# markokr/libacm

Measured on AMD Instinct MI355X. Metric: decoded PCM Msamples/sec over a batch of ACM streams (hot path on HBM-resident staged input), higher is better.
Workload: dtype int32

## Files before the change

### libacm_amd/csrc/acm_kernels.hip

```cpp
#include <hip/hip_runtime.h>

#include <utility>

#include "acm_device.h"

#ifndef ACM_L14_GROUPS
#define ACM_L14_GROUPS 3, 3, 3, 3, 2
#endif
#ifndef ACM_L13_GROUPS
#define ACM_L13_GROUPS 2, 3, 3, 3, 2
#endif

#ifndef ACM_OUT_F32
#define ACM_OUT_F32 0
#endif
#if ACM_OUT_F32
#define ACM_K_EMIT acm_sw_emit_f32
#define ACM_K_SMALL acm_small_level_f32
#define ACM_K_FUSED acm_fused_tile_f32
#define ACM_K_TILE2 acm_f32_tile2
#define ACM_K_CHUNK acm_f32_chunk
#define ACMK_OUT(name) name##_f32
#else
#define ACM_K_EMIT acm_sw_emit
#define ACM_K_SMALL acm_small_level
#define ACM_K_FUSED acm_fused_tile
#define ACM_K_TILE2 acm_tile2
#define ACM_K_CHUNK acm_chunk
#define ACMK_OUT(name) name
#endif

namespace {

__device__ __forceinline__ uint32_t pcm16(int32_t v, int level, unsigned fmt)
{
	uint32_t w = (uint32_t)(v >> level);
	if (fmt & 2u)
		w += 0x8000u;
	w &= 0xFFFFu;
	if (fmt & 1u)
		w = ((w & 0xFFu) << 8) | (w >> 8);
	return w;
}

typedef float v2f __attribute__((ext_vector_type(2)));
typedef float v4f __attribute__((ext_vector_type(4)));

__device__ __forceinline__ v2f pcm_pair_f32(uint32_t w)
{
	const v2f f = { (float)(int32_t)(int16_t)(w & 0xFFFFu), (float)((int32_t)w >> 16) };
	return f * 0x1p-15f;
}

__device__ __forceinline__ v4f pcm_quad_f32(uint32_t a, uint32_t b)
{
	const v2f x = pcm_pair_f32(a), y = pcm_pair_f32(b);
	return v4f{ x.x, x.y, y.x, y.y };
}

__device__ __forceinline__ float pcm_one_f32(int32_t v, int level)
{
	return (float)(int32_t)(int16_t)(uint16_t)pcm16(v, level, ACMHIP_FMT_S16LE) * 0x1p-15f;
}

constexpr int SW_THREADS = 256;

#if !ACM_OUT_F32
__global__ void __launch_bounds__(SW_THREADS)
acm_sw_unpack(const AcmDevStream *__restrict__ streams, const uint32_t *__restrict__ list,
	      const int16_t *__restrict__ idx, const acmhip_blkhdr *__restrict__ hdr,
	      int32_t *__restrict__ x, const uint32_t shift)
{
	const AcmDevStream s = streams[list[blockIdx.y]];
	const uint64_t first = (uint64_t)s.halo_row << s.level;
	const uint64_t n = ((uint64_t)(s.nrows - s.halo_row)) << s.level;
	const int16_t *src = idx + s.idx_off + first;
	const acmhip_blkhdr *h = hdr + s.hdr_off;
	int32_t *dst = x + s.scratch_off;
	for (uint64_t e = (uint64_t)blockIdx.x * SW_THREADS + threadIdx.x; e < n;
	     e += (uint64_t)gridDim.x * SW_THREADS) {
		const uint32_t row = s.halo_row + (uint32_t)(e >> s.level);
		const uint32_t val = h[row / s.rows].val;
		dst[e] = (int32_t)((uint32_t)(int32_t)src[e] * (val << shift));
	}
}

__global__ void __launch_bounds__(SW_THREADS)
// ... 1878 lines not shown
			return (i & 3u) + CB * ((i >> 2) & 1u) + 4u * (i >> 3);
	}

	struct Raw { v4u_t lo[NG][NX], hi[NG][NX]; };
	struct Desc { uint32_t e[NE]; };
	struct Tables {
		v4i_t coef[3][NM][64];
		int32_t bias[3][2][QN];
		int32_t rsum[3][QN];
	};

	static __device__ __forceinline__ void fill_tables(Tables &t, const int tid, const int nthreads)
	{
		constexpr int32_t ONE = 1 << OutScale<L>::SHIFT;
		for (int k = tid; k < 3 * NM * 64; k += nthreads) {
			const int j = k / (NM * 64), mt = (k / 64) % NM, lane = k % 64;
			t.coef[j][mt][lane] = *reinterpret_cast<const v4i_t *>(&ACM_TZ6[VARIANT][j][16 * mt + (lane & 15)][16 * (lane >> 4)]);
		}
		for (int k = tid; k < 3 * 2 * QN; k += nthreads) {
			const int var = k / (2 * QN), par = (k / QN) & 1, q = k % QN;
			t.bias[var][par][q] = par ? 0 : ACM_TZ6_BIAS[VARIANT][var][q] * ONE;
		}
		for (int k = tid; k < 3 * QN; k += nthreads) {
			int32_t sum = 0;
			for (int c = 0; c < 64; c++)
				sum += ACM_TZ6[VARIANT][k / QN][k % QN][c];
			t.rsum[k / QN][k % QN] = 128 * sum;
		}
	}

	static __device__ __forceinline__ Desc fetch_desc(const uint32_t *__restrict__ pairs, const AcmTile2 &r)
	{
		Desc d;
		const uint32_t at = __builtin_amdgcn_readfirstlane((uint32_t)r.idx_off);
#pragma unroll
		for (int j = 0; j < NE; j++)
			d.e[j] = pairs[at + j];
		return d;
	}

	static __device__ __forceinline__ uint32_t entry_of(const Desc &d, const uint32_t u)
	{
		uint32_t e = (uint32_t)opaque_s((int32_t)d.e[0]);
#pragma unroll
		for (int j = 1; j < NE; j++)
			e = (u >> 1) >= (uint32_t)j ? (uint32_t)opaque_s((int32_t)d.e[j]) : e;
		return e;
	}

	static constexpr bool HISTORY_IN_REGISTERS = RR == 1;
#ifndef ACM_K3_DPP_HISTORY
#define ACM_K3_DPP_HISTORY 1
#endif
	static constexpr bool HISTORY_BY_DPP = ACM_K3_DPP_HISTORY && RR >= 2 && NSW == 2 && RR * SIGMA == 16 && SIGMA >= 4;
	static constexpr bool KEEPS_ROWS = HISTORY_IN_REGISTERS || HISTORY_BY_DPP;
	template <int CTRL, int BANKS>
	static __device__ __forceinline__ v4u_t dpp4(const v4u_t old, const v4u_t src)
	{
		v4u_t r;
#pragma unroll
		for (int v = 0; v < 4; v++)
			r[v] = (uint32_t)__builtin_amdgcn_update_dpp((int)old[v], (int)src[v], CTRL, 0xF, BANKS, false);
		return r;
	}
	static constexpr int DPP_W0_BANKS = (1 << (SIGMA / 4)) - 1;
	static __device__ __forceinline__ void hand_history_on(Raw &raw)
	{
#pragma unroll
		for (int k = 0; k < 2; k++) {
			raw.lo[0][k] = dpp4<0x100 + (16 - SIGMA), DPP_W0_BANKS>(raw.lo[0][k], raw.lo[0][k + NSW]);
			raw.hi[0][k] = dpp4<0x100 + (16 - SIGMA), DPP_W0_BANKS>(raw.hi[0][k], raw.hi[0][k + NSW]);
		}
	}
	static __device__ __forceinline__ void take_history_from_partner(Raw &raw)
	{
#pragma unroll
		for (int k = 0; k < 2; k++) {
			raw.lo[0][k] = dpp4<0x110 + SIGMA, 0xF & ~DPP_W0_BANKS>(raw.lo[0][k], raw.lo[0][k + NSW]);
			raw.hi[0][k] = dpp4<0x110 + SIGMA, 0xF & ~DPP_W0_BANKS>(raw.hi[0][k], raw.hi[0][k + NSW]);
		}
	}
	static constexpr int JM = (TR & 1) ? 1 : TR / 2;
	static_assert(JM + 1 <= NE, "entries in reach are entries fetched");
	static __device__ __forceinline__ uint32_t half_bytes(const uint32_t cls) { return (0x4234u >> (4u * cls)) & 15u; }
	template <int J0>
	static __device__ __forceinline__ uint32_t mode_of(const uint32_t flags, const Desc &d, const uint32_t sval)
	{
		const uint32_t cls = d.e[0] & 3u;
		const uint32_t pair_units = (uint32_t)(COLS / 64) * half_bytes(cls);
		bool ok = (flags & ACM_TILE_ONEBLOCK) != 0 && cls != 0u;
		if constexpr (OutScale<L>::SHIFT != 0)
			ok = ok && sval < 65536u;
#pragma unroll
		for (int j = 1; j <= JM; j++)
			ok = ok && (d.e[j] & 3u) == cls;
#pragma unroll
		for (int j = J0; j < JM; j++)
			ok = ok && (d.e[j + 1] >> 2) - (d.e[j] >> 2) == pair_units;
		return ok ? (cls == ACMHIP_BP_NIB12 ? 3u : cls - (ACMHIP_BP_BYTE - 1u)) : 0u;
	}

#ifndef ACM_K3_LD_MOD
#define ACM_K3_LD_MOD " nt"
#endif
	template <bool KEEP>
	static __device__ __forceinline__ void issue(Raw &raw, const uint8_t *arena, const Desc &d, const int lane, const uint32_t odd, const uint32_t mode)
	{
		static_assert(!KEEP || KEEPS_ROWS, "the rows in front belong to another lane");
		constexpr int K0 = KEEP ? 2 : 0, J0 = KEEP ? 1 : 0;
		const uint32_t i = (uint32_t)lane & 15u, ks = (uint32_t)lane >> 4;
		const uint32_t c = class_of(i), rr = RR == 1 ? 0u : i / SIGMA;
		const uint32_t smode = __builtin_amdgcn_readfirstlane(mode);
		uint32_t va[NX][NG], vh[NX][NG];
		const uint8_t *sb[NX][NG];
		if (mode) {
			const uint32_t hb = smode == 1u ? 2u : smode == 2u ? 4u : 3u;
			const uint64_t base = reinterpret_cast<uint64_t>(arena) + ((uint64_t)(d.e[J0] >> 2) << 6);
			const uint32_t vl = (rr * (uint32_t)(NSW * COLS / 2) + c * (uint32_t)(QN / 2)) * hb + 16u * ks;
			const uint32_t vlh = vl - (smode == 3u ? 8u * ks : 0u);
#pragma unroll
			for (int k = K0; k < NX; k++)
#pragma unroll
				for (int g = 0; g < NG; g++) {
					va[k][g] = vl;
					vh[k][g] = vlh;
					sb[k][g] = sgpr_u64(base + (uint64_t)((((TR & 1 ? odd : 0u) + (uint32_t)(k - K0)) * (uint32_t)(COLS / 2) + group_at(g) * (uint32_t)(QN / 2)) * hb));
				}
		} else {
			const uint32_t e0 = d.e[0];
			const uint8_t *base = sgpr_u64(reinterpret_cast<uint64_t>(arena) + ((uint64_t)(e0 >> 2) << 6));
#pragma unroll
			for (int k = K0; k < NX; k++) {
				const uint32_t u = (TR & 1 ? odd : 0u) + rr * NSW + k;
				const uint32_t e = entry_of(d, u);
				const uint32_t hb = half_bytes(e & 3u);
				const uint32_t row_at = (((e >> 2) - (e0 >> 2)) << 6) + ((u & 1u) ? (uint32_t)(COLS / 2) * hb : 0u) + 16u * ks;
#pragma unroll
				for (int g = 0; g < NG; g++) {
					va[k][g] = row_at + (group_at(g) + c) * (uint32_t)(QN / 2) * hb;
					vh[k][g] = va[k][g] - ((e & 3u) == ACMHIP_BP_NIB12 ? 8u * ks : 0u);
					sb[k][g] = base;
				}
			}
		}
#pragma unroll
		for (int k = K0; k < NX; k++)
#pragma unroll
			for (int g = 0; g < NG; g++) {
				if constexpr (KEEPS_ROWS) {
					asm volatile("global_load_dwordx4 %0, %1, %2" ACM_K3_LD_MOD : "=v"(raw.lo[g][k]) : "v"(va[k][g]), "s"(sb[k][g]) : "memory");
					asm volatile("s_cmp_eq_u32 %3, 1\n\ts_cbranch_scc1 .Lacm_z8_%=\n\t"
						     "global_load_dwordx4 %0, %1, %2 offset:64" ACM_K3_LD_MOD "\n"
						     ".Lacm_z8_%=:"
						     : "+v"(raw.hi[g][k]) : "v"(vh[k][g]), "s"(sb[k][g]), "s"(smode) : "memory", "scc");
				} else {
					asm volatile("global_load_dwordx4 %0, %1, %2" : "=v"(raw.lo[g][k]) : "v"(va[k][g]), "s"(sb[k][g]) : "memory");
					asm volatile("s_cmp_eq_u32 %3, 1\n\ts_cbranch_scc1 .Lacm_z8_%=\n\t"
						     "global_load_dwordx4 %0, %1, %2 offset:64\n"
						     ".Lacm_z8_%=:"
						     : "+v"(raw.hi[g][k]) : "v"(vh[k][g]), "s"(sb[k][g]), "s"(smode) : "memory", "scc");
				}
			}
	}
	static __device__ __forceinline__ v4u_t expand_nib(const v4u_t x)
	{
		const uint32_t M = 0xF0F0F0F0u;
		return v4u_t{ x[0] & M, (x[0] << 4) & M, x[1] & M, (x[1] << 4) & M };
	}
	static __device__ __forceinline__ v4u_t sra4(const v4u_t x)
	{
		v4u_t r;
#pragma unroll
		for (int v = 0; v < 4; v++) {
			const uint32_t m = x[v] & 0x80808080u;
			r[v] = ((x[v] >> 4) & 0x0F0F0F0Fu) | ((m << 1) - (m >> 3));
		}
		return r;
	}
	static __device__ __forceinline__ v4u_t shl4(const v4u_t x)
	{
		return v4u_t{ (x[0] << 4) & 0xF0F0F0F0u, (x[1] << 4) & 0xF0F0F0F0u, (x[2] << 4) & 0xF0F0F0F0u, (x[3] << 4) & 0xF0F0F0F0u };
	}
	static __device__ __forceinline__ void shift_history(Raw &raw)
	{
#pragma unroll
		for (int g = 0; g < NG; g++)
#pragma unroll
			for (int k = 0; k < 2; k++) {
				raw.lo[g][k] = raw.lo[g][k + NSW];
				raw.hi[g][k] = raw.hi[g][k + NSW];
			}
	}
	static __device__ __forceinline__ void zero_history(Raw &raw)
	{
		const v4u_t z = { 0, 0, 0, 0 };
#pragma unroll
		for (int g = 0; g < NG; g++)
#pragma unroll
			for (int k = 0; k < 2; k++)
				raw.lo[g][k] = raw.hi[g][k] = z;
	}

	static __device__ __forceinline__ v4i_t mfma(const v4u_t data, const v4i_t coef, const v4i_t acc)
	{
		return __builtin_amdgcn_mfma_i32_16x16x64_i8((v4i_t)data, coef, acc, 0, 0, 0);
	}

	static __device__ __forceinline__ int32_t opaque_s(int32_t v)
	{
		asm("" : "+s"(v));
		return v;
	}
	static __device__ __forceinline__ int32_t opaque_v(int32_t v)
	{
		asm("" : "+v"(v));
		return v;
	}

	template <bool WORDS, bool FAST, bool NIB = false>
	static __device__ __forceinline__ void run_t(const Raw &raw, uint32_t *const tile, const Tables &t, const int lane, const uint32_t hvs,
						     const uint32_t in_front, const uint32_t sval, const bool wordu = false, const Desc *dd = nullptr,
						     const uint32_t odd = 0u, const bool nform = false)
	{
		static_assert(!NIB || (WORDS && FAST), "rows in N form are a fast-path matter; the general path takes them to bytes first");
		const v4i_t zero = { 0, 0, 0, 0 };
		const uint32_t h = (uint32_t)lane >> 4, qd = (uint32_t)lane & 15u;
		uint32_t c0[NH], rrd[NH];
		uint32_t o_lane[NH];
#pragma unroll
		for (int hf = 0; hf < NH; hf++) {
			const uint32_t i = 4u * h + (uint32_t)(hf * NVH);
			c0[hf] = RR == 1 ? class_of(i) : i % SIGMA;
			rrd[hf] = RR == 1 ? 0u : i / SIGMA;
			const uint32_t m_lane = rrd[hf] * (uint32_t)(NSW * COLS) + c0[hf] + (uint32_t)SIGMA * qd;
			o_lane[hf] = m_lane + (m_lane >> PS);
		}
		uint32_t bias_at[NSW][NH];
		int32_t val[NSW][NH], dv2[NSW][NH], dv1[NSW][NH];
		bool step2[NSW], step1[NSW];
		bool small[NSW];
#pragma unroll
		for (int s = 0; s < NSW; s++)
			small[s] = OutScale<L>::SHIFT == 0;
		if constexpr (FAST) {
#pragma unroll
			for (int s = 0; s < NSW; s++) {
				step2[s] = step1[s] = false;
				small[s] = true;
#pragma unroll
				for (int hf = 0; hf < NH; hf++)
					val[s][hf] = dv2[s][hf] = dv1[s][hf] = 0;
			}
		} else if constexpr (RR <= 2) {
			int32_t rowval[TR + 2];
#pragma unroll
			for (int k = 0; k < TR + 2; k++)
				rowval[k] = (int32_t)__builtin_amdgcn_readlane(hvs, k);
#pragma unroll
			for (int s = 0; s < NSW; s++) {
				const int32_t a0 = rowval[s + 2], a1 = rowval[s + 1], a2 = rowval[s];
				if constexpr (RR == 1) {
					val[s][0] = a0;
					dv2[s][0] = a1 - a0;
					dv1[s][0] = a2 - a1;
					step2[s] = a1 != a0;
					step1[s] = a2 != a1;
					small[s] = (uint32_t)a0 < 65536u;
				} else {
					const int32_t b0 = rowval[NSW + s + 2], b1 = rowval[NSW + s + 1], b2 = rowval[NSW + s];
					val[s][0] = rrd[0] ? b0 : a0;
					dv2[s][0] = rrd[0] ? b1 - b0 : a1 - a0;
					dv1[s][0] = rrd[0] ? b2 - b1 : a2 - a1;
					step2[s] = a1 != a0 || b1 != b0;
					step1[s] = a2 != a1 || b2 != b1;
					small[s] = (uint32_t)(a0 | b0) < 65536u;
				}
			}
		} else {
			const uint32_t first = (uint32_t)__builtin_amdgcn_readfirstlane(hvs);
			const bool one_val = __builtin_amdgcn_ballot_w64(lane < TR + 2 && hvs != first) == 0;
#pragma unroll
			for (int s = 0; s < NSW; s++)
				step2[s] = step1[s] = false;
#pragma unroll
			for (int hf = 0; hf < NH; hf++) {
				int32_t g[NSW + 2];
#pragma unroll
				for (int k = 0; k < NSW + 2; k++)
					g[k] = one_val ? (int32_t)first : __builtin_amdgcn_ds_bpermute((int)(4u * (rrd[hf] * NSW + (uint32_t)k)), (int32_t)hvs);
#pragma unroll
				for (int s = 0; s < NSW; s++) {
					val[s][hf] = g[s + 2];
					dv2[s][hf] = g[s + 1] - g[s + 2];
					dv1[s][hf] = g[s] - g[s + 1];
					if (!one_val) {
						step2[s] = step2[s] || __builtin_amdgcn_ballot_w64(dv2[s][hf] != 0) != 0;
						step1[s] = step1[s] || __builtin_amdgcn_ballot_w64(dv1[s][hf] != 0) != 0;
					}
				}
			}
		}
#pragma unroll
		for (int s = 0; s < NSW; s++)
#pragma unroll
			for (int hf = 0; hf < NH; hf++) {
				const uint32_t row = in_front + rrd[hf] * NSW + s;
				bias_at[s][hf] = ((row < 2 ? row : 2u) * 2u + (c0[hf] == 0 ? 0u : 1u)) * (uint32_t)QN + qd;
			}
		const v4i_t *cf = &t.coef[0][0][lane];
		const auto &hi = raw.hi;
#ifndef ACM_K3_MT_UNROLL
#define ACM_K3_MT_UNROLL 1
#endif
#define ACM_PRAGMA_(x) _Pragma(#x)
#define ACM_UNROLL(n) ACM_PRAGMA_(unroll n)
		ACM_UNROLL(ACM_K3_MT_UNROLL)
		for (int mt = 0; mt < NM; mt++) {
			const v4i_t cf0 = cf[0], cf1 = cf[NM * 64], cf2 = cf[2 * NM * 64];
#pragma unroll
			for (int e = 0; e < NSET; e++) {
				const int g = e / NSW, s = e % NSW;
				int32_t b[NH];
#pragma unroll
				for (int hf = 0; hf < NH; hf++)
					b[hf] = g == 0 ? (&t.bias[0][0][0])[bias_at[s][hf] + 16u * (uint32_t)mt] : 0;
				const v4i_t l1 = mfma(raw.lo[g][s], cf2, zero);
				const v4i_t l2 = mfma(raw.lo[g][s + 1], cf1, l1);
				const v4i_t la = mfma(raw.lo[g][s + 2], cf0, l2);
				v4i_t y;
				if constexpr (FAST) {
					const int32_t sv = opaque_s((int32_t)__builtin_amdgcn_readfirstlane(sval));
#pragma unroll
					for (int v = 0; v < 4; v++)
						y[v] = __mul24(la[v], sv) + (v % NVH == 0 ? b[v / NVH] : 0);
					if constexpr (WORDS) {
						const v4i_t h1 = mfma(hi[g][s], cf2, zero);
						const v4i_t h2 = mfma(hi[g][s + 1], cf1, h1);
						const v4i_t ha = mfma(hi[g][s + 2], cf0, h2);
						if constexpr (NIB) {
							const int32_t sv4 = opaque_s((int32_t)__builtin_amdgcn_readfirstlane(sval << 4));
#pragma unroll
							for (int v = 0; v < 4; v++)
								y[v] = __mul24(ha[v], sv4) + y[v];
						} else {
							const uint32_t sv8 = (uint32_t)opaque_s((int32_t)__builtin_amdgcn_readfirstlane(sval << 8));
#pragma unroll
							for (int v = 0; v < 4; v++)
								y[v] = (int32_t)(__umul24((uint32_t)ha[v], sv8) + (uint32_t)y[v]);
						}
					}
				} else {
#pragma unroll
				for (int v = 0; v < 4; v++)
					y[v] = __mul24(la[v], val[s][v / NVH]) + (v % NVH == 0 ? b[v / NVH] : 0);
				if (step2[s]) {
#pragma unroll
					for (int v = 0; v < 4; v++)
						y[v] += __mul24(l2[v], dv2[s][v / NVH]);
				}
				if (step1[s]) {
#pragma unroll
					for (int v = 0; v < 4; v++)
						y[v] += __mul24(l1[v], dv1[s][v / NVH]);
				}
				if constexpr (WORDS && NH == 1) {
					if (wordu) {
						const int32_t *rs = &t.rsum[0][0] + 16 * mt + (int)qd;
						bool urow[3];
#pragma unroll
						for (int j = 0; j < 3; j++)
							urow[j] = (entry_of(*dd, (TR & 1 ? odd : 0u) + rrd[0] * NSW + (uint32_t)(s + j)) & 3u) == ACMHIP_BP_WORDU;
						const int32_t v0 = val[s][0], v1 = v0 + dv2[s][0], v2 = v1 + dv1[s][0];
						const int32_t add = __mul24(urow[2] ? v0 : 0, rs[0]) + __mul24(urow[1] ? v1 : 0, rs[QN]) + __mul24(urow[0] ? v2 : 0, rs[2 * QN]);
#pragma unroll
						for (int v = 0; v < 4; v++)
							y[v] += add;
					}
				}
				if constexpr (WORDS) {
					const v4i_t h1 = mfma(hi[g][s], cf2, zero);
					const v4i_t h2 = mfma(hi[g][s + 1], cf1, h1);
					const v4i_t ha = mfma(hi[g][s + 2], cf0, h2);
					{
						if (small[s] && !step2[s] && !step1[s] && !nform) {
							uint32_t v8[NH];
#pragma unroll
							for (int hf = 0; hf < NH; hf++)
								v8[hf] = (uint32_t)opaque_v((int32_t)((uint32_t)val[s][hf] << 8));
#pragma unroll
							for (int v = 0; v < 4; v++)
								y[v] = (int32_t)(__umul24((uint32_t)ha[v], v8[v / NVH]) + (uint32_t)y[v]);
							goto joined;
						}
					}
					{
					v4i_t yh;
					int32_t wv[NH], w2[NH], w1[NH];
#pragma unroll
					for (int hf = 0; hf < NH; hf++) {
						wv[hf] = opaque_v(val[s][hf]);
						w2[hf] = opaque_v(dv2[s][hf]);
						w1[hf] = opaque_v(dv1[s][hf]);
					}
#pragma unroll
					for (int v = 0; v < 4; v++)
						yh[v] = __mul24(ha[v], wv[v / NVH]);
					if (step2[s]) {
#pragma unroll
						for (int v = 0; v < 4; v++)
							yh[v] += __mul24(h2[v], w2[v / NVH]);
					}
					if (step1[s]) {
#pragma unroll
						for (int v = 0; v < 4; v++)
							yh[v] += __mul24(h1[v], w1[v / NVH]);
					}
					const uint32_t hs = nform ? 4u : 8u;
#pragma unroll
					for (int v = 0; v < 4; v++)
						y[v] = (int32_t)(((uint32_t)opaque_v(yh[v]) << hs) + (uint32_t)y[v]);
					}
				joined:;
				}
				}
				static_assert(COLS % (1 << PS) == 0 && (SIGMA * 16) % (1 << PS) == 0 &&
					      (NG == 1 || (group_at(NG - 1) % (1 << PS) + CB + 7 < (1 << PS) && SIGMA % (1 << PS) == 0)), "address split");
#pragma unroll
				for (int hf = 0; hf < NH; hf++) {
					uint32_t *const o = tile + (o_lane[hf] + (uint32_t)((s * COLS + ((s * COLS) >> PS)) + (group_at(g) + (group_at(g) >> PS))));
#pragma unroll
					for (int v = 0; v < NVH; v++)
						o[v] = (uint32_t)y[hf * NVH + v];
				}
			}
			cf += 64;
#pragma unroll
			for (int hf = 0; hf < NH; hf++)
				o_lane[hf] += SIGMA * 16 + ((SIGMA * 16) >> PS);
		}
	}

	static __device__ __forceinline__ void run(Raw &raw, uint32_t *const tile, const Tables &t, const int lane_, const uint32_t hvs,
						   const Desc &d, const uint32_t in_front, const uint32_t odd, const uint32_t mode, const uint32_t sval,
						   const bool first)
	{
#ifdef ACM_K3_OPAQUE_LANE
		const int lane = opaque_v(lane_);
#else
		const int lane = lane_;
#endif
		const bool all_new = !KEEPS_ROWS || first;
		if (mode == 3u) {
#pragma unroll
			for (int k = 0; k < NX; k++)
				if (k >= 2 || all_new) {
#pragma unroll
					for (int g = 0; g < NG; g++)
						raw.hi[g][k] = expand_nib(raw.hi[g][k]);
				}
			if constexpr (HISTORY_BY_DPP)
				take_history_from_partner(raw);
			run_t<true, true, true>(raw, tile, t, lane, 0u, in_front, sval);
			return;
		}
		if (mode) {
			if constexpr (HISTORY_BY_DPP)
				take_history_from_partner(raw);
			if (mode == 2u)
				run_t<true, true>(raw, tile, t, lane, 0u, in_front, sval);
			else
				run_t<false, true>(raw, tile, t, lane, 0u, in_front, sval);
			return;
		}
		uint32_t any_word = 0, any_nib = 0, any_wordu = 0;
#pragma unroll
		for (int j = 0; j < NE; j++) {
			any_word |= (d.e[j] & 3u) == ACMHIP_BP_WORD ? 1u : 0u;
			any_nib |= (d.e[j] & 3u) == ACMHIP_BP_NIB12 ? 1u : 0u;
			any_wordu |= (d.e[j] & 3u) == ACMHIP_BP_WORDU ? 1u : 0u;
		}
		any_word |= any_wordu;
		const uint32_t rr = RR == 1 ? 0u : ((uint32_t)lane & 15u) / SIGMA;
		if (any_nib) {
#pragma unroll
			for (int k = 0; k < NX; k++)
				if (k >= 2 || all_new) {
					if ((entry_of(d, (TR & 1 ? odd : 0u) + rr * NSW + k) & 3u) == ACMHIP_BP_NIB12) {
#pragma unroll
						for (int g = 0; g < NG; g++)
							raw.hi[g][k] = expand_nib(raw.hi[g][k]);
					}
				}
		}
		if constexpr (HISTORY_BY_DPP)
			take_history_from_partner(raw);
		const bool nform = any_nib && !any_word;
		if (any_word | any_nib) {
#pragma unroll
			for (int k = 0; k < NX; k++) {
				const uint32_t cls = entry_of(d, (TR & 1 ? odd : 0u) + rr * NSW + k) & 3u;
				const uint32_t mask = cls == ACMHIP_BP_BYTE ? 0u : 0xFFFFFFFFu;
#pragma unroll
				for (int g = 0; g < NG; g++)
					raw.hi[g][k] &= mask;
				if (any_nib && !nform && cls == ACMHIP_BP_NIB12) {
#pragma unroll
					for (int g = 0; g < NG; g++)
						raw.hi[g][k] = sra4(raw.hi[g][k]);
				}
			}
			run_t<true, false>(raw, tile, t, lane, hvs, in_front, 0u, any_wordu != 0, &d, odd, nform);
			if (any_nib && !nform && KEEPS_ROWS) {
#pragma unroll
				for (int k = NSW; k < NX; k++)
					if ((entry_of(d, (TR & 1 ? odd : 0u) + rr * NSW + k) & 3u) == ACMHIP_BP_NIB12) {
#pragma unroll
						for (int g = 0; g < NG; g++)
							raw.hi[g][k] = shl4(raw.hi[g][k]);
					}
			}
		} else {
			run_t<false, false>(raw, tile, t, lane, hvs, in_front, 0u);
		}
	}
};

template <int L_, int ABL, int... Gs>
__global__ void __launch_bounds__(64 * FirstPassZ<L_>::NW, 1)
ACM_K_CHUNK(const AcmTile2 *__restrict__ tiles, const uint32_t ntiles, const int16_t *__restrict__ idx, const uint32_t *__restrict__ pairs,
	  const acmhip_blkhdr *__restrict__ hdr, int16_t *__restrict__ pcm, int16_t *__restrict__ sink, const unsigned fmt)
{
	constexpr bool F32 = ACM_OUT_F32;

	using FP = FirstPassZ<L_>;
	using C = typename FP::C;
	constexpr int L = L_, COLS = C::COLS, NELEM = C::NELEM, TR = C::TR, NJ_LAST = C::NJ_LAST, NW = FP::NW;
	constexpr int WTILE = 8 + NELEM + (NELEM >> C::PS);
	constexpr int NCARRY_WORDS = carry_total<C, FP::G, Gs...>();
	constexpr int PASS_ABL = ABL | MODE_WAVE | (FP::NG > 1 && NW == 16 ? MODE_LEAN : 0);

	__shared__ uint32_t tile_mem[NW][WTILE];
	__shared__ uint32_t carry_all[NW][NCARRY_WORDS];
	__shared__ typename FP::Tables tables;

	const int lane0 = threadIdx.x & 63;
	const uint32_t wave = __builtin_amdgcn_readfirstlane(threadIdx.x >> 6);
	FP::fill_tables(tables, threadIdx.x, NW * 64);
	__syncthreads();

	uint32_t *const tile = tile_mem[wave] + 8;
	uint32_t *const carry_mem = carry_all[wave];

	const uint32_t nvw = gridDim.x * NW, vw = blockIdx.x * NW + wave;
	const uint32_t per = (ntiles + nvw - 1) / nvw;
	uint32_t t = vw * per;
	const uint32_t t_end = t + per < ntiles ? t + per : ntiles;
	if (t >= t_end)
		return;
	bool discard = false;
	{
		const uint32_t f0 = tiles[__builtin_amdgcn_readfirstlane(t)].flags;
		if (f0 & ACM_TILE_DISCARD) {
			discard = true;
		} else if (!(f0 & ACM_TILE_FRESH)) {
			discard = true;
			t--;
		}
	}

	auto rows_in_front = [](const AcmTile2 &r) -> uint32_t { return (r.flags & ACM_TILE_FRESH) ? 0u : (r.flags & ACM_TILE_ROW1) ? 1u : 2u; };
	auto fetch_val = [&](const AcmTile2 &r, const int lane, uint32_t v, const uint32_t mode) -> uint32_t {
		const uint32_t *p = &hdr[0].val;
		if (!mode) {
			const uint32_t lr_fetch = (uint32_t)(lane < TR + 2 ? lane : TR + 1);
			const uint32_t missing = 2u - rows_in_front(r);
			const uint32_t q = r.rowpos + (lr_fetch < missing ? 0u : lr_fetch - missing);
			const uint32_t b = r.magic ? __umulhi(q, r.magic) : q;
			p = &hdr[r.hdr_blk + b].val;
		}
		asm volatile("s_cmp_lg_u32 %2, 0\n\ts_cbranch_scc1 .Lacm_zv_%=\n\t"
			     "global_load_dword %0, %1, off\n"
			     ".Lacm_zv_%=:"
			     : "+v"(v) : "v"(p), "s"(__builtin_amdgcn_readfirstlane(mode)) : "memory", "scc");
		return v;
	};
	typedef const uint32_t __attribute__((address_space(4))) *const_u32_ptr;
	auto val_of = [&](const AcmTile2 &r) -> uint32_t {
		const uint64_t a = reinterpret_cast<uint64_t>(&hdr[__builtin_amdgcn_readfirstlane(r.hdr_blk)].val);
		return *(const_u32_ptr)a << OutScale<L>::SHIFT;
	};

	constexpr int NVEC = TR * COLS / 8, PER_OWNER = NJ_LAST / 8, NSTORE = NVEC / 64;
	static_assert(NVEC % 64 == 0, "whole rounds");
	const uint8_t *const arena = reinterpret_cast<const uint8_t *>(idx);
	auto record_at = [&](const uint32_t k) -> AcmTile2 { return tiles[__builtin_amdgcn_readfirstlane(k < t_end ? k : t_end - 1)]; };
	constexpr int MODE_J0 = FP::KEEPS_ROWS ? 1 : 0;
#ifdef ACM_K3_NO_FAST
	auto mode_of = [&](const AcmTile2 &, const typename FP::Desc &, const uint32_t) -> uint32_t { return 0u; };
#else
	auto mode_of = [&](const AcmTile2 &r, const typename FP::Desc &d, const uint32_t sval) -> uint32_t {
		return FP::template mode_of<MODE_J0>(r.flags, d, sval);
	};
#endif
	AcmTile2 cur = record_at(t);
	typename FP::Desc dcur = FP::fetch_desc(pairs, cur);
	typename FP::Raw raw;
	{
		const v4u_t z = { 0, 0, 0, 0 };
#pragma unroll
		for (int g = 0; g < FP::NG; g++)
#pragma unroll
			for (int k = 0; k < FP::NX; k++)
				raw.hi[g][k] = z;
	}
	uint32_t mode_cur = 0u, sv_cur = val_of(cur);
	uint32_t hv = fetch_val(cur, lane0, 0u, 0u);
	FP::template issue<false>(raw, arena, dcur, lane0, (cur.flags & ACM_TILE_ODD) ? 1u : 0u, 0u);
	k2_wait<0>();
	bool fresh = true, first_of_run = true;
	AcmTile2 nxt = record_at(t + 1), nx2 = record_at(t + 2);
	typename FP::Desc dnxt = FP::fetch_desc(pairs, nxt);
	uint32_t sv_nxt = val_of(nxt);
	uint32_t mode_nxt = mode_of(nxt, dnxt, sv_nxt);
#ifdef ACM_STAMPS
	unsigned long long acc_[8] = { 0, 0, 0, 0, 0, 0, 0, 0 };
	unsigned long long last_ = stamp_now();
#endif
	for (;;) {
		const uint32_t tn = t + 1;
		const bool more = tn < t_end;
		int lane = lane0;
#ifdef ACM_K3_OPAQUE_LANE
		asm volatile("" : "+v"(lane));
#endif
		if (fresh)
			for (int k = lane; k < NCARRY_WORDS; k += 64)
				carry_mem[k] = 0u;
		const uint32_t hvs = hv << OutScale<L>::SHIFT;
		ACM_STAMP(0);
		phase_prio<true, PRIO_FIRST_PASS>();
		FP::run(raw, tile, tables, lane, hvs, dcur, rows_in_front(cur), (cur.flags & ACM_TILE_ODD) ? 1u : 0u, mode_cur, sv_cur, first_of_run);
		first_of_run = false;
		phase_prio<true, PRIO_IDLE>();
		ACM_STAMP(1);

		hv = fetch_val(nxt, lane, hv, mode_nxt);
		if constexpr (FP::HISTORY_IN_REGISTERS) {
			FP::shift_history(raw);
			if (nxt.flags & ACM_TILE_FRESH)
				FP::zero_history(raw);
			FP::template issue<true>(raw, arena, dnxt, lane, (nxt.flags & ACM_TILE_ODD) ? 1u : 0u, mode_nxt);
		} else if constexpr (FP::HISTORY_BY_DPP) {
			FP::hand_history_on(raw);
			if (nxt.flags & ACM_TILE_FRESH)
				FP::zero_history(raw);
			FP::template issue<true>(raw, arena, dnxt, lane, (nxt.flags & ACM_TILE_ODD) ? 1u : 0u, mode_nxt);
		} else {
			FP::template issue<false>(raw, arena, dnxt, lane, (nxt.flags & ACM_TILE_ODD) ? 1u : 0u, mode_nxt);
		}
		const AcmTile2 nx3 = record_at(t + 3);
		const typename FP::Desc dnx2 = FP::fetch_desc(pairs, nx2);
		const uint32_t sv_nx2 = val_of(nx2);
		ACM_STAMP(2);
		phase_prio<true, PRIO_LDS_PASSES>();
		run_lds_passes<C, PASS_ABL, true, FP::G, Gs...>(tile, lane, F32 ? (unsigned)ACMHIP_FMT_S16LE : fmt, carry_mem);
		tile_barrier<MODE_WAVE>();
		ACM_STAMP(3);
		if constexpr (F32) {
			float *out = discard ? reinterpret_cast<float *>(sink) : reinterpret_cast<float *>(pcm) + cur.pcm_off;
			lean_store_f32<C, 64, NSTORE, ABL>(tile, lane, out);
		} else {
			typedef uint32_t v4u __attribute__((ext_vector_type(4)));
			v4u *out = discard ? reinterpret_cast<v4u *>(sink) : reinterpret_cast<v4u *>(reinterpret_cast<uint16_t *>(pcm) + cur.pcm_off);
#pragma unroll
			for (int k = 0; k < NSTORE; k++) {
				const int vec = lane + k * 64;
				const uint32_t *q = tile + lds_at<C::PS>((vec / PER_OWNER) * NJ_LAST) + (vec % PER_OWNER) * park_piece<NJ_LAST>();
				const v4u o = { q[0], q[1], q[2], q[3] };
#ifdef ACM_K3_ST_MOD
				asm volatile("global_store_dwordx4 %0, %1, %2" ACM_K3_ST_MOD :: "v"((uint32_t)(vec * 16)), "v"(o), "s"(sgpr_u64(reinterpret_cast<uint64_t>(out))) : "memory");
#else
				__builtin_nontemporal_store(o, &out[vec]);
#endif
			}
		}
		ACM_STAMP(5);
		phase_prio<true, PRIO_IDLE>();
		k2_wait<F32 ? 2 * NSTORE : NSTORE>();
		ACM_STAMP(6);
		tile_barrier<MODE_WAVE>();
		if (!more)
			break;
		fresh = (nxt.flags & (ACM_TILE_FRESH | ACM_TILE_DISCARD)) != 0;
		discard = (nxt.flags & ACM_TILE_DISCARD) != 0;
		cur = nxt;
		dcur = dnxt;
		sv_cur = sv_nxt;
		mode_cur = mode_nxt;
		t = tn;
		nxt = nx2;
		dnxt = dnx2;
		sv_nxt = sv_nx2;
		mode_nxt = mode_of(nxt, dnxt, sv_nxt);
		nx2 = nx3;
	}
#ifdef ACM_STAMPS
	if (lane0 == 0 && vw < 2048)
		for (int k = 0; k < 8; k++)
			g_acm_stamps[vw][k] = acc_[k];
#endif
}

struct Tile2Entry {
	typedef void (*Fn)(const AcmTile2 *, uint32_t, const int16_t *, const uint32_t *, const acmhip_blkhdr *, int16_t *, int16_t *, unsigned);
	Fn fn;
	int threads, tile_rows, wg_per_cu;
};
template <class C, int... Gs>
constexpr Tile2Entry entry_k2()
{
	return Tile2Entry{ ACM_K_TILE2<C, 4, 0, false, Gs...>, C::NT, C::TR, 1024 / C::NT };
}
template <class C, int WPC, int... Gs>
constexpr Tile2Entry entry_k2w()
{
	return Tile2Entry{ ACM_K_TILE2<C, WPC * C::NT / 256, 0, false, Gs...>, C::NT, C::TR, WPC };
}
#ifdef ACM_ABLATION
template <int ABL>
constexpr Tile2Entry abl_k2() { return Tile2Entry{ ACM_K_TILE2<TileCfg<9, 256, 8192>, 4, ABL, false, 3, 3, 3>, 256, 16, 4 }; }
const struct { int mask; Tile2Entry e; } g_tile2_abl[] = {
	{ 1, abl_k2<1>() }, { 2, abl_k2<2>() }, { 4, abl_k2<4>() }, { 6, abl_k2<6>() }, { 8, abl_k2<8>() }, { 16, abl_k2<16>() },
	{ 17, abl_k2<17>() }, { 23, abl_k2<23>() }, { 32, abl_k2<32>() }, { 25, abl_k2<25>() }, { 31, abl_k2<31>() }, { 12, abl_k2<12>() },
};
#endif
const Tile2Entry g_tile2[ACM_K2_MAX_LEVEL - ACM_K2_MIN_LEVEL + 1] = {
	entry_k2<TileCfg<6, 256, 8192>, 2, 2, 2>(),
	entry_k2<TileCfg<7, 256, 8192>, 3, 2, 2>(),
	entry_k2<TileCfg<8, 256, 8192>, 3, 3, 2>(),
	entry_k2<TileCfg<9, 256, 8192>, 3, 3, 3>(),
	entry_k2<TileCfg<10, 256, 8192>, 3, 3, 2, 2>(),
	entry_k2<TileCfg<11, 256, 8192>, 3, 3, 3, 2>(),
	entry_k2w<TileCfg<12, 512, 16384>, 2, 3, 3, 3, 3>(),
	entry_k2w<TileCfg<13, 1024, 32768>, 1, ACM_L13_GROUPS>(),
	entry_k2w<TileCfg<14, 1024, 32768>, 1, ACM_L14_GROUPS>(),
};
inline const Tile2Entry &tile2_entry(uint32_t level)
{
	return g_tile2[level - ACM_K2_MIN_LEVEL];
}
template <class C, int... Gs>
constexpr Tile2Entry entry_k2m()
{
	return Tile2Entry{ ACM_K_TILE2<C, 4, 0, true, Gs...>, C::NT, C::TR, 1024 / C::NT };
}
template <class C, int WPC, int... Gs>
constexpr Tile2Entry entry_k2mw()
{
	return Tile2Entry{ ACM_K_TILE2<C, WPC * C::NT / 256, 0, true, Gs...>, C::NT, C::TR, WPC };
}
#ifndef ACM_K2M_L11
#define ACM_K2M_L11 entry_k2m<TileCfg<11, 256, 8192>, 4, 3, 2, 2>(), 4
#endif
#ifndef ACM_K2M_L12
#define ACM_K2M_L12 entry_k2mw<TileCfg<12, 512, 16384>, 2, 4, 3, 3, 2>(), 4
#endif
#ifndef ACM_K2M_L13
#define ACM_K2M_L13 entry_k2mw<TileCfg<13, 512, 16384>, 2, 4, 3, 3, 3>(), 4
#endif
struct Tile2MEntry { Tile2Entry e; int g0; };
#ifdef ACM_TUNING
#define ACM_K2M_ALT(...) __VA_ARGS__
#else
#define ACM_K2M_ALT(...) Tile2Entry{ nullptr, 0, 0, 0 }, 0
#endif
const Tile2MEntry g_tile2m[ACM_K2M_MAX_LEVEL - ACM_K2M_MIN_LEVEL + 1][2] = {
	{ { entry_k2m<TileCfg<7, 256, 8192>, 3, 2, 2>(), 3 }, { Tile2Entry{ nullptr, 0, 0, 0 }, 0 } },
	{ { entry_k2m<TileCfg<8, 256, 8192>, 3, 3, 2>(), 3 }, { ACM_K2M_ALT(entry_k2m<TileCfg<8, 256, 8192>, 4, 2, 2>(), 4) } },
	{ { entry_k2m<TileCfg<9, 256, 8192>, 3, 3, 3>(), 3 }, { ACM_K2M_ALT(entry_k2m<TileCfg<9, 256, 8192>, 4, 3, 2>(), 4) } },
	{ { ACM_K2M_ALT(entry_k2m<TileCfg<10, 256, 8192>, 3, 3, 2, 2>(), 3) }, { entry_k2m<TileCfg<10, 256, 8192>, 4, 3, 3>(), 4 } },
	{ { ACM_K2M_ALT(entry_k2m<TileCfg<11, 256, 8192>, 3, 3, 3, 2>(), 3) }, { ACM_K2M_L11 } },
	{ { ACM_K2M_ALT(entry_k2mw<TileCfg<12, 512, 16384>, 2, 3, 3, 3, 3>(), 3) }, { ACM_K2M_L12 } },
	{ { Tile2Entry{ nullptr, 0, 0, 0 }, 0 }, { ACM_K2M_L13 } },
	{ { Tile2Entry{ nullptr, 0, 0, 0 }, 0 }, { entry_k2mw<TileCfg<14, 1024, 32768>, 1, 4, 2, 3, 3, 2>(), 4 } },
};
// ... 489 lines not shown
}

extern "C" int acmk_tile2_grid(uint32_t level, int cus)
{
	if (level < ACM_K2_MIN_LEVEL || level > ACM_K2_MAX_LEVEL)
		return 0;
	return (cus > 0 ? cus : 256) * tile2_entry(level).wg_per_cu;
}

#endif
extern "C" int ACMK_OUT(acmk_launch_tile2)(uint32_t level, int cus, const AcmTile2 *d_tiles, uint32_t ntiles, const int16_t *d_idx, const acmhip_blkhdr *d_hdr,
				 int16_t *d_pcm, int16_t *d_sink, unsigned fmt, void *stream)
{
#if !ACM_OUT_F32
	if (fmt & ACMK_FMT_F32)
		return acmk_launch_tile2_f32(level, cus, d_tiles, ntiles, d_idx, d_hdr, d_pcm, d_sink, fmt & 3u, stream);
#endif
	if (ntiles == 0)
		return 0;
	if (!d_sink)
		return -1;
	if (level < ACM_K2_MIN_LEVEL || level > ACM_K2_MAX_LEVEL)
		return -1;
	Tile2Entry e = tile2_entry(level);
#ifdef ACM_ABLATION
	if (const char *a = getenv("ACM_K2_ABL"))
		for (const auto &x : g_tile2_abl)
			if (level == 9 && x.mask == atoi(a))
				e = x.e;
#endif
	uint32_t grid = (uint32_t)((cus > 0 ? cus : 256) * e.wg_per_cu);
	if (grid > ntiles)
		grid = ntiles;
	hipLaunchKernelGGL(e.fn, dim3(grid), dim3(e.threads), 0, (hipStream_t)stream, d_tiles, ntiles, d_idx, (const uint32_t *)nullptr, d_hdr, d_pcm, d_sink, fmt);
	ACMK_CHECK_LAUNCH();
	return 0;
}

#if !ACM_OUT_F32
extern "C" int acmk_tile2m_rows(uint32_t level)
{
	if (level < ACM_K2M_MIN_LEVEL || level > ACM_K2M_MAX_LEVEL)
		return 0;
	return tile2m_entry(level).e.tile_rows;
}

extern "C" int acmk_tile2m_lead_in(uint32_t level)
{
	if (level < ACM_K2M_MIN_LEVEL || level > ACM_K2M_MAX_LEVEL || tile2m_entry(level).g0 != 6)
		return 1;
	switch (level) {
	case 8: return FirstPassZ<8>::KEEPS_ROWS ? 1 + (2 + FirstPassZ<8>::NSW - 1) / FirstPassZ<8>::NSW : 1;
	case 9: return FirstPassZ<9>::KEEPS_ROWS ? 1 + (2 + FirstPassZ<9>::NSW - 1) / FirstPassZ<9>::NSW : 1;
	case 10: return FirstPassZ<10>::HISTORY_IN_REGISTERS ? 1 + (2 + FirstPassZ<10>::NSW - 1) / FirstPassZ<10>::NSW : 1;
	case 11: return FirstPassZ<11>::HISTORY_IN_REGISTERS ? 1 + (2 + FirstPassZ<11>::NSW - 1) / FirstPassZ<11>::NSW : 1;
	case 12: return FirstPassZ<12>::HISTORY_IN_REGISTERS ? 1 + (2 + FirstPassZ<12>::NSW - 1) / FirstPassZ<12>::NSW : 1;
	case 13: case 14: return 2;
	default: return 1;
	}
}

extern "C" int acmk_tile2m_run_waves(uint32_t level, int cus)
{
	if (level < ACM_K2M_MIN_LEVEL || level > 12 || tile2m_entry(level).g0 != 6)
		return 0;
	const Tile2Entry &e = tile2m_entry(level).e;
	return (cus > 0 ? cus : 256) * e.wg_per_cu * (e.threads / 64);
}

extern "C" int acmk_tile2m_grid(uint32_t level, int cus)
{
	if (level < ACM_K2M_MIN_LEVEL || level > ACM_K2M_MAX_LEVEL)
		return 0;
	return (cus > 0 ? cus : 256) * tile2m_entry(level).e.wg_per_cu;
}

extern "C" int acmk_tile2m_stages(uint32_t level)
{
	if (level < ACM_K2M_MIN_LEVEL || level > ACM_K2M_MAX_LEVEL)
		return 0;
	return tile2m_entry(level).g0;
}

#endif
extern "C" int ACMK_OUT(acmk_launch_tile2m)(uint32_t level, int cus, const AcmTile2 *d_tiles, uint32_t ntiles, const uint8_t *d_mform, const acmhip_mform_pair *d_pairs,
				  const acmhip_blkhdr *d_hdr, int16_t *d_pcm, int16_t *d_sink, unsigned fmt, void *stream)
{
#if !ACM_OUT_F32
	if (fmt & ACMK_FMT_F32)
		return acmk_launch_tile2m_f32(level, cus, d_tiles, ntiles, d_mform, d_pairs, d_hdr, d_pcm, d_sink, fmt & 3u, stream);
#endif
	if (ntiles == 0)
		return 0;
	if (!d_sink || !d_mform || !d_pairs)
		return -1;
	if (level < ACM_K2M_MIN_LEVEL || level > ACM_K2M_MAX_LEVEL)
		return -1;
	const Tile2Entry &e = tile2m_entry(level).e;
	uint32_t grid = (uint32_t)((cus > 0 ? cus : 256) * e.wg_per_cu);
	if (grid > ntiles)
		grid = ntiles;
	hipLaunchKernelGGL(e.fn, dim3(grid), dim3(e.threads), 0, (hipStream_t)stream, d_tiles, ntiles, reinterpret_cast<const int16_t *>(d_mform),
			   reinterpret_cast<const uint32_t *>(d_pairs), d_hdr, d_pcm, d_sink, fmt);
	ACMK_CHECK_LAUNCH();
	return 0;
}

#if !ACM_OUT_F32
extern "C" int acmk_tile2p_rows(uint32_t level)
{
	if (level < ACM_K2P_MIN_LEVEL || level > ACM_K2P_MAX_LEVEL)
		return 0;
	return g_tile2p[level - ACM_K2P_MIN_LEVEL].tile_rows;
}

extern "C" int acmk_tile2p_group_rows(uint32_t level)
{
	if (level < ACM_K2P_MIN_LEVEL || level > ACM_K2P_MAX_LEVEL)
		return 0;
	return g_tile2p[level - ACM_K2P_MIN_LEVEL].group_rows;
}

extern "C" int acmk_tile2p_slots(uint32_t level)
{
	if (level < ACM_K2P_MIN_LEVEL || level > ACM_K2P_MAX_LEVEL)
		return 0;
	return g_tile2p[level - ACM_K2P_MIN_LEVEL].slots;
}

extern "C" int acmk_tile2p_waves(uint32_t level)
{
	if (level < ACM_K2P_MIN_LEVEL || level > ACM_K2P_MAX_LEVEL)
		return 0;
	return g_tile2p[level - ACM_K2P_MIN_LEVEL].threads / 64;
}

extern "C" int acmk_tile2p_pad_shift(uint32_t level)
{
	if (level < ACM_K2P_MIN_LEVEL || level > ACM_K2P_MAX_LEVEL)
		return 0;
	return g_tile2p[level - ACM_K2P_MIN_LEVEL].pad_shift;
}

extern "C" int acmk_launch_tile2p(uint32_t level, int cus, const AcmTile2 *d_tiles, uint32_t ntiles, const acmhip_packed_chunk *d_chunks, const uint8_t *d_blob,
				  const acmhip_blkhdr *d_hdr, int16_t *d_pcm, int16_t *d_sink, unsigned fmt, void *stream)
{
	if (ntiles == 0)
		return 0;
	if (!d_sink || !d_chunks || !d_blob)
		return -1;
	if (level < ACM_K2P_MIN_LEVEL || level > ACM_K2P_MAX_LEVEL)
		return -1;
	const Tile2PEntry &e = g_tile2p[level - ACM_K2P_MIN_LEVEL];
	uint32_t grid = (uint32_t)((cus > 0 ? cus : 256) * e.wg_per_cu);
	if (grid > ntiles)
		grid = ntiles;
	static_assert(sizeof(acmhip_packed_chunk) == sizeof(uint2), "a chunk descriptor is two words");
	hipLaunchKernelGGL(e.fn, dim3(grid), dim3(e.threads), 0, (hipStream_t)stream, d_tiles, ntiles, reinterpret_cast<const uint2 *>(d_chunks), d_blob, d_hdr,
			   d_pcm, d_sink, fmt);
	ACMK_CHECK_LAUNCH();
	return 0;
}

extern "C" int acmk_plane_tile_rows(void)
{
	return g_fused_plane.tile_rows;
// ... 46 lines not shown
```

Before: 1.457 million.

## Add stepped fast path for tiles straddling two blocks in first pass

Adds a new fast mode (ACM_CHUNK_STEPPED) for non-oneblock tiles whose rows cross exactly one block boundary. Those tiles previously fell back to the general path. The new path runs MFMA-based reconstruction with two block scales (sval and sval2), splitting the history contribution by walker. It also templates run_t on the packing classes of both blocks. Mode selection moves into a shared host/device header, and a host query entry point is added. The cost is a per-tile extra header load (val2_of) and more template instantiations, which adds code size and register pressure.

```diff
diff --git a/libacm_amd/csrc/acm_chunk_mode.h b/libacm_amd/csrc/acm_chunk_mode.h
--- /dev/null
+++ b/libacm_amd/csrc/acm_chunk_mode.h
@@ -0,0 +1,61 @@
+#ifndef ACM_CHUNK_MODE_H
+#define ACM_CHUNK_MODE_H
+
+#include <stdint.h>
+
+#include "acm_device.h"
+
+#if defined(__HIPCC__) || defined(__CUDACC__)
+#define ACM_CHUNK_MODE_FN __host__ __device__ inline
+#else
+#define ACM_CHUNK_MODE_FN inline
+#endif
+
+#define ACM_CHUNK_STEPPED 4u
+
+ACM_CHUNK_MODE_FN uint32_t acm_bp_half_bytes(const uint32_t cls) { return (0x4234u >> (4u * cls)) & 15u; }
+ACM_CHUNK_MODE_FN uint32_t acm_chunk_fast_mode(const uint32_t cls) { return cls == ACMHIP_BP_NIB12 ? 3u : cls - (ACMHIP_BP_BYTE - 1u); }
+ACM_CHUNK_MODE_FN uint32_t acm_chunk_block_of(const uint32_t q, const uint32_t magic)
+{
+	return magic ? (uint32_t)(((uint64_t)q * magic) >> 32) : q;
+}
+
+template <int COLS, int JM>
+ACM_CHUNK_MODE_FN bool acm_chunk_one_width(const uint32_t *e, const int j_class, const int j_place, const uint32_t cls)
+{
+	const uint32_t pair_units = (uint32_t)(COLS / 64) * acm_bp_half_bytes(cls);
+	bool ok = true;
+#pragma unroll
+	for (int j = j_class; j <= JM; j++)
+		ok = ok && (e[j] & 3u) == cls;
+#pragma unroll
+	for (int j = j_place; j < JM; j++)
+		ok = ok && (e[j + 1] >> 2) - (e[j] >> 2) == pair_units;
+	return ok;
+}
+
+template <int TR, int COLS, int JM, int J0, bool SCALED, bool STEPS>
+ACM_CHUNK_MODE_FN uint32_t acm_chunk_mode(const uint32_t flags, const uint32_t rowpos, const uint32_t magic, const uint32_t *e, const uint32_t sval)
+{
+	const uint32_t cls = e[0] & 3u;
+	if (flags & ACM_TILE_ONEBLOCK) {
+		bool ok = cls != ACMHIP_BP_WORDU && (!SCALED || sval < 65536u);
+		ok = ok && acm_chunk_one_width<COLS, JM>(e, 1, J0, cls);
+		return ok ? acm_chunk_fast_mode(cls) : 0u;
+	}
+	if (!STEPS || (flags & (ACM_TILE_FRESH | ACM_TILE_ROW1 | ACM_TILE_ODD)))
+		return 0u;
+	if ((rowpos + 2u) % (uint32_t)TR != 0u || acm_chunk_block_of(rowpos + 1u, magic) != 0u || acm_chunk_block_of(rowpos + 2u, magic) != 1u ||
+	    acm_chunk_block_of(rowpos + 2u + (uint32_t)TR - 1u, magic) != 1u)
+		return 0u;
+	const uint32_t own = e[1] & 3u;
+	if (cls == ACMHIP_BP_WORDU || own == ACMHIP_BP_WORDU || !acm_chunk_one_width<COLS, JM>(e, 2, 1, own))
+		return 0u;
+	return ACM_CHUNK_STEPPED + acm_chunk_fast_mode(own);
+}
+
+extern "C" {
+int acmk_chunk_mode(uint32_t level, uint32_t flags, uint32_t rowpos, uint32_t magic, const uint32_t *entries, uint32_t sval);
+}
+
+#endif
diff --git a/libacm_amd/csrc/acm_kernels.hip b/libacm_amd/csrc/acm_kernels.hip
--- a/libacm_amd/csrc/acm_kernels.hip
+++ b/libacm_amd/csrc/acm_kernels.hip
@@ -3,6 +3,7 @@
 #include <utility>
 
 #include "acm_device.h"
+#include "acm_chunk_mode.h"
 
 #ifndef ACM_L14_GROUPS
 #define ACM_L14_GROUPS 3, 3, 3, 3, 2
@@ -2047,22 +2048,12 @@
 	}
 	static constexpr int JM = (TR & 1) ? 1 : TR / 2;
 	static_assert(JM + 1 <= NE, "entries in reach are entries fetched");
-	static __device__ __forceinline__ uint32_t half_bytes(const uint32_t cls) { return (0x4234u >> (4u * cls)) & 15u; }
+	static __device__ __forceinline__ uint32_t half_bytes(const uint32_t cls) { return acm_bp_half_bytes(cls); }
+	static constexpr bool STEPS = RR == 2 && NSW == 2 && HISTORY_BY_DPP;
 	template <int J0>
-	static __device__ __forceinline__ uint32_t mode_of(const uint32_t flags, const Desc &d, const uint32_t sval)
-	{
-		const uint32_t cls = d.e[0] & 3u;
-		const uint32_t pair_units = (uint32_t)(COLS / 64) * half_bytes(cls);
-		bool ok = (flags & ACM_TILE_ONEBLOCK) != 0 && cls != 0u;
-		if constexpr (OutScale<L>::SHIFT != 0)
-			ok = ok && sval < 65536u;
-#pragma unroll
-		for (int j = 1; j <= JM; j++)
-			ok = ok && (d.e[j] & 3u) == cls;
-#pragma unroll
-		for (int j = J0; j < JM; j++)
-			ok = ok && (d.e[j + 1] >> 2) - (d.e[j] >> 2) == pair_units;
-		return ok ? (cls == ACMHIP_BP_NIB12 ? 3u : cls - (ACMHIP_BP_BYTE - 1u)) : 0u;
+	static __host__ __device__ __forceinline__ uint32_t mode_of(const uint32_t flags, const uint32_t rowpos, const uint32_t magic, const Desc &d, const uint32_t sval)
+	{
+		return acm_chunk_mode<TR, COLS, JM, J0, OutScale<L>::SHIFT != 0, STEPS>(flags, rowpos, magic, d.e, sval);
 	}
 
 #ifndef ACM_K3_LD_MOD
@@ -2182,12 +2173,14 @@
 		return v;
 	}
 
-	template <bool WORDS, bool FAST, bool NIB = false>
+	template <bool WORDS, bool FAST, bool NIB = false, int HA = -1, int HB = 0>
 	static __device__ __forceinline__ void run_t(const Raw &raw, uint32_t *const tile, const Tables &t, const int lane, const uint32_t hvs,
 						     const uint32_t in_front, const uint32_t sval, const bool wordu = false, const Desc *dd = nullptr,
-						     const uint32_t odd = 0u, const bool nform = false)
-	{
+						     const uint32_t odd = 0u, const bool nform = false, const uint32_t sval2 = 0u)
+	{
+		constexpr bool STEP = HA >= 0;
 		static_assert(!NIB || (WORDS && FAST), "rows in N form are a fast-path matter; the general path takes them to bytes first");
+		static_assert(!STEP || (FAST && !NIB && STEPS && NH == 1 && WORDS == (HA + HB != 0)), "the stepped path: two walkers of two rows, scalars throughout");
 		const v4i_t zero = { 0, 0, 0, 0 };
 		const uint32_t h = (uint32_t)lane >> 4, qd = (uint32_t)lane & 15u;
 		uint32_t c0[NH], rrd[NH];
@@ -2274,6 +2267,8 @@
 			}
 		const v4i_t *cf = &t.coef[0][0][lane];
 		const auto &hi = raw.hi;
+		[[maybe_unused]] const int32_t step_w0 = STEP ? opaque_v(rrd[0] == 0u ? -1 : 0) : 0;
+		[[maybe_unused]] const int32_t step_dv = STEP ? opaque_v((int32_t)(sval - sval2) & step_w0) : 0;
 #ifndef ACM_K3_MT_UNROLL
 #define ACM_K3_MT_UNROLL 1
 #endif
@@ -2293,7 +2288,40 @@
 				const v4i_t l2 = mfma(raw.lo[g][s + 1], cf1, l1);
 				const v4i_t la = mfma(raw.lo[g][s + 2], cf0, l2);
 				v4i_t y;
-				if constexpr (FAST) {
+				if constexpr (STEP) {
+					const int32_t svb = opaque_s((int32_t)__builtin_amdgcn_readfirstlane(sval2));
+					const v4i_t &pl = s == 0 ? l2 : l1;
+#pragma unroll
+					for (int v = 0; v < 4; v++)
+						y[v] = __mul24(pl[v], step_dv) + (v == 0 ? b[0] : 0);
+#pragma unroll
+					for (int v = 0; v < 4; v++)
+						y[v] = __mul24(la[v], svb) + y[v];
+					if constexpr (WORDS) {
+						const v4i_t h1 = mfma(hi[g][s], cf2, zero);
+						const v4i_t ph = s == 0 ? mfma(hi[g][s + 1], cf1, h1) : h1;
+						v4i_t pe, rest;
+#pragma unroll
+						for (int v = 0; v < 4; v++) {
+							pe[v] = ph[v] & step_w0;
+							rest[v] = ph[v] ^ pe[v];
+						}
+						if constexpr (HA != 0) {
+							const int32_t ma = opaque_s((int32_t)__builtin_amdgcn_readfirstlane(sval << (HA == 1 ? 4 : 8)));
+#pragma unroll
+							for (int v = 0; v < 4; v++)
+								y[v] = HA == 1 ? __mul24(pe[v], ma) + y[v] : (int32_t)(__umul24((uint32_t)pe[v], (uint32_t)ma) + (uint32_t)y[v]);
+						}
+						if constexpr (HB != 0) {
+							const v4i_t h2 = s == 0 ? rest : mfma(hi[g][s + 1], cf1, rest);
+							const v4i_t hd = mfma(hi[g][s + 2], cf0, h2);
+							const int32_t mb = opaque_s((int32_t)__builtin_amdgcn_readfirstlane(sval2 << (HB == 1 ? 4 : 8)));
+#pragma unroll
+							for (int v = 0; v < 4; v++)
+								y[v] = HB == 1 ? __mul24(hd[v], mb) + y[v] : (int32_t)(__umul24((uint32_t)hd[v], (uint32_t)mb) + (uint32_t)y[v]);
+						}
+					}
+				} else if constexpr (FAST) {
 					const int32_t sv = opaque_s((int32_t)__builtin_amdgcn_readfirstlane(sval));
 #pragma unroll
 					for (int v = 0; v < 4; v++)
@@ -2407,7 +2435,7 @@
 
 	static __device__ __forceinline__ void run(Raw &raw, uint32_t *const tile, const Tables &t, const int lane_, const uint32_t hvs,
 						   const Desc &d, const uint32_t in_front, const uint32_t odd, const uint32_t mode, const uint32_t sval,
-						   const bool first)
+						   const bool first, const uint32_t sval2 = 0u)
 	{
 #ifdef ACM_K3_OPAQUE_LANE
 		const int lane = opaque_v(lane_);
@@ -2415,6 +2443,43 @@
 		const int lane = lane_;
 #endif
 		const bool all_new = !KEEPS_ROWS || first;
+		if constexpr (STEPS) {
+			if (mode & ACM_CHUNK_STEPPED) {
+				if ((mode & 3u) == 3u) {
+#pragma unroll
+					for (int k = 2; k < NX; k++)
+						raw.hi[0][k] = expand_nib(raw.hi[0][k]);
+				}
+				take_history_from_partner(raw);
+				const uint32_t ca = d.e[0] & 3u;
+				const uint32_t own = mode & 3u;
+#define ACM_STEP_RUN(ha, hb) run_t<((ha) + (hb) != 0), true, false, ha, hb>(raw, tile, t, lane, 0u, in_front, sval, false, nullptr, 0u, false, sval2)
+				if (own == 1u) {
+					if (ca == ACMHIP_BP_BYTE)
+						ACM_STEP_RUN(0, 0);
+					else if (ca == ACMHIP_BP_NIB12)
+						ACM_STEP_RUN(1, 0);
+					else
+						ACM_STEP_RUN(2, 0);
+				} else if (own == 3u) {
+					if (ca == ACMHIP_BP_BYTE)
+						ACM_STEP_RUN(0, 1);
+					else if (ca == ACMHIP_BP_NIB12)
+						ACM_STEP_RUN(1, 1);
+					else
+						ACM_STEP_RUN(2, 1);
+				} else {
+					if (ca == ACMHIP_BP_BYTE)
+						ACM_STEP_RUN(0, 2);
+					else if (ca == ACMHIP_BP_NIB12)
+						ACM_STEP_RUN(1, 2);
+					else
+						ACM_STEP_RUN(2, 2);
+				}
+#undef ACM_STEP_RUN
+				return;
+			}
+		}
 		if (mode == 3u) {
 #pragma unroll
 			for (int k = 0; k < NX; k++)
@@ -2564,9 +2629,18 @@
 	auto mode_of = [&](const AcmTile2 &, const typename FP::Desc &, const uint32_t) -> uint32_t { return 0u; };
 #else
 	auto mode_of = [&](const AcmTile2 &r, const typename FP::Desc &d, const uint32_t sval) -> uint32_t {
-		return FP::template mode_of<MODE_J0>(r.flags, d, sval);
+		return FP::template mode_of<MODE_J0>(r.flags, r.rowpos, r.magic, d, sval);
 	};
 #endif
+	auto val2_of = [&](const AcmTile2 &r) -> uint32_t {
+		if constexpr (FP::STEPS) {
+			const uint32_t blk = __builtin_amdgcn_readfirstlane(r.hdr_blk) + ((r.flags & ACM_TILE_ONEBLOCK) ? 0u : 1u);
+			const uint64_t a = reinterpret_cast<uint64_t>(&hdr[blk].val);
+			return *(const_u32_ptr)a << OutScale<L>::SHIFT;
+		} else {
+			return 0u;
+		}
+	};
 	AcmTile2 cur = record_at(t);
 	typename FP::Desc dcur = FP::fetch_desc(pairs, cur);
 	typename FP::Raw raw;
@@ -2578,14 +2652,14 @@
 			for (int k = 0; k < FP::NX; k++)
 				raw.hi[g][k] = z;
 	}
-	uint32_t mode_cur = 0u, sv_cur = val_of(cur);
+	uint32_t mode_cur = 0u, sv_cur = val_of(cur), sb_cur = 0u;
 	uint32_t hv = fetch_val(cur, lane0, 0u, 0u);
 	FP::template issue<false>(raw, arena, dcur, lane0, (cur.flags & ACM_TILE_ODD) ? 1u : 0u, 0u);
 	k2_wait<0>();
 	bool fresh = true, first_of_run = true;
 	AcmTile2 nxt = record_at(t + 1), nx2 = record_at(t + 2);
 	typename FP::Desc dnxt = FP::fetch_desc(pairs, nxt);
-	uint32_t sv_nxt = val_of(nxt);
+	uint32_t sv_nxt = val_of(nxt), sb_nxt = val2_of(nxt);
 	uint32_t mode_nxt = mode_of(nxt, dnxt, sv_nxt);
 #ifdef ACM_STAMPS
 	unsigned long long acc_[8] = { 0, 0, 0, 0, 0, 0, 0, 0 };
@@ -2604,7 +2678,7 @@
 		const uint32_t hvs = hv << OutScale<L>::SHIFT;
 		ACM_STAMP(0);
 		phase_prio<true, PRIO_FIRST_PASS>();
-		FP::run(raw, tile, tables, lane, hvs, dcur, rows_in_front(cur), (cur.flags & ACM_TILE_ODD) ? 1u : 0u, mode_cur, sv_cur, first_of_run);
+		FP::run(raw, tile, tables, lane, hvs, dcur, rows_in_front(cur), (cur.flags & ACM_TILE_ODD) ? 1u : 0u, mode_cur, sv_cur, first_of_run, sb_cur);
 		first_of_run = false;
 		phase_prio<true, PRIO_IDLE>();
 		ACM_STAMP(1);
@@ -2614,18 +2688,18 @@
 			FP::shift_history(raw);
 			if (nxt.flags & ACM_TILE_FRESH)
 				FP::zero_history(raw);
-			FP::template issue<true>(raw, arena, dnxt, lane, (nxt.flags & ACM_TILE_ODD) ? 1u : 0u, mode_nxt);
+			FP::template issue<true>(raw, arena, dnxt, lane, (nxt.flags & ACM_TILE_ODD) ? 1u : 0u, mode_nxt & 3u);
 		} else if constexpr (FP::HISTORY_BY_DPP) {
 			FP::hand_history_on(raw);
 			if (nxt.flags & ACM_TILE_FRESH)
 				FP::zero_history(raw);
-			FP::template issue<true>(raw, arena, dnxt, lane, (nxt.flags & ACM_TILE_ODD) ? 1u : 0u, mode_nxt);
+			FP::template issue<true>(raw, arena, dnxt, lane, (nxt.flags & ACM_TILE_ODD) ? 1u : 0u, mode_nxt & 3u);
 		} else {
-			FP::template issue<false>(raw, arena, dnxt, lane, (nxt.flags & ACM_TILE_ODD) ? 1u : 0u, mode_nxt);
+			FP::template issue<false>(raw, arena, dnxt, lane, (nxt.flags & ACM_TILE_ODD) ? 1u : 0u, mode_nxt & 3u);
 		}
 		const AcmTile2 nx3 = record_at(t + 3);
 		const typename FP::Desc dnx2 = FP::fetch_desc(pairs, nx2);
-		const uint32_t sv_nx2 = val_of(nx2);
+		const uint32_t sv_nx2 = val_of(nx2), sb_nx2 = val2_of(nx2);
 		ACM_STAMP(2);
 		phase_prio<true, PRIO_LDS_PASSES>();
 		run_lds_passes<C, PASS_ABL, true, FP::G, Gs...>(tile, lane, F32 ? (unsigned)ACMHIP_FMT_S16LE : fmt, carry_mem);
@@ -2661,11 +2735,13 @@
 		cur = nxt;
 		dcur = dnxt;
 		sv_cur = sv_nxt;
+		sb_cur = sb_nxt;
 		mode_cur = mode_nxt;
 		t = tn;
 		nxt = nx2;
 		dnxt = dnx2;
 		sv_nxt = sv_nx2;
+		sb_nxt = sb_nx2;
 		mode_nxt = mode_of(nxt, dnxt, sv_nxt);
 		nx2 = nx3;
 	}
@@ -3321,6 +3397,29 @@
 	return tile2m_entry(level).g0;
 }
 
+template <int L>
+static int chunk_mode_at(uint32_t flags, uint32_t rowpos, uint32_t magic, const uint32_t *entries, uint32_t sval)
+{
+	using FP = FirstPassZ<L>;
+	typename FP::Desc d = {};
+	for (int j = 0; j <= FP::JM; j++)
+		d.e[j] = entries[j];
+	return (int)FP::template mode_of<FP::KEEPS_ROWS ? 1 : 0>(flags, rowpos, magic, d, sval);
+}
+extern "C" int acmk_chunk_mode(uint32_t level, uint32_t flags, uint32_t rowpos, uint32_t magic, const uint32_t *entries, uint32_t sval)
+{
+	if (!entries)
+		return -1;
+	switch (level) {
+	case 8: return chunk_mode_at<8>(flags, rowpos, magic, entries, sval);
+	case 9: return chunk_mode_at<9>(flags, rowpos, magic, entries, sval);
+	case 10: return chunk_mode_at<10>(flags, rowpos, magic, entries, sval);
+	case 11: return chunk_mode_at<11>(flags, rowpos, magic, entries, sval);
+	case 12: return chunk_mode_at<12>(flags, rowpos, magic, entries, sval);
+	default: return -1;
+	}
+}
+
 #endif
 extern "C" int ACMK_OUT(acmk_launch_tile2m)(uint32_t level, int cus, const AcmTile2 *d_tiles, uint32_t ntiles, const uint8_t *d_mform, const acmhip_mform_pair *d_pairs,
 				  const acmhip_blkhdr *d_hdr, int16_t *d_pcm, int16_t *d_sink, unsigned fmt, void *stream)
```

After: 1.374 million. 0.943x the previous value.
